# Hxyz-123/GoMatching

Measured on AMD Instinct MI355X. Metric: frames/sec (whole node), 1280x720 clip, 100 queries/frame, higher is better.
Workload: dtype f32 (f16x3 split MFMA: 22-bit significand products, fp32 accumulate; parity tests at fp32 tolerances)

## Files before the change

gomatching_amd/csrc/msda.hip:

```cpp
#include <mutex>
#include <type_traits>
#include <vector>

#include "common.h"

namespace {

constexpr int HEADS = 8, CH = 32, LEVELS = 4;

__device__ __forceinline__ long xcd_contiguous_block(unsigned bid, unsigned nwg) {
    const unsigned q = nwg >> 3, r = nwg & 7, xcd = bid & 7;
    return (long)(xcd < r ? xcd * (q + 1) : r * (q + 1) + (xcd - r) * q) + (bid >> 3);
}

template <int POINTS>
__global__ __launch_bounds__(256) void msda_fwd_kernel(const float* __restrict__ value,
                                                       const int64_t* __restrict__ shapes,
                                                       const int64_t* __restrict__ lsi,
                                                       const float* __restrict__ loc,
                                                       const float* __restrict__ attw, float* __restrict__ out,
                                                       int B, int Lq, long v_bs, int v_rs) {
    const long q_global = xcd_contiguous_block(blockIdx.x, gridDim.x) * 4 + (threadIdx.x >> 6);
    if (q_global >= (long)B * Lq) return;
    const int lane = threadIdx.x & 63;
// ... 247 lines not shown

    const __amdgpu_buffer_rsrc_t rs = gom_buffer_rsrc(value + (size_t)b * v_bs, 0x7FFFFFFF);
    const unsigned mine = (unsigned)k * 16u;
    f32x4 acc = {0.f, 0.f, 0.f, 0.f};
#pragma unroll
    for (int i = 0; i < LP; ++i) {
        const int o = i >> 1, t = i & 1;
        const unsigned a1 = __builtin_bit_cast(unsigned, group8_read(__builtin_bit_cast(float, so1[t]), o)) + mine;
        const unsigned a2 = __builtin_bit_cast(unsigned, group8_read(__builtin_bit_cast(float, so2[t]), o)) + mine;
        const unsigned a3 = __builtin_bit_cast(unsigned, group8_read(__builtin_bit_cast(float, so3[t]), o)) + mine;
        const unsigned a4 = __builtin_bit_cast(unsigned, group8_read(__builtin_bit_cast(float, so4[t]), o)) + mine;
        const f32x4 v1 = __builtin_bit_cast(f32x4, __builtin_amdgcn_raw_buffer_load_b128(rs, (int)a1, 0, 0));
        const f32x4 v2 = __builtin_bit_cast(f32x4, __builtin_amdgcn_raw_buffer_load_b128(rs, (int)a2, 0, 0));
        const f32x4 v3 = __builtin_bit_cast(f32x4, __builtin_amdgcn_raw_buffer_load_b128(rs, (int)a3, 0, 0));
        const f32x4 v4 = __builtin_bit_cast(f32x4, __builtin_amdgcn_raw_buffer_load_b128(rs, (int)a4, 0, 0));
        const float w1 = group8_read(sw1[t], o), w2 = group8_read(sw2[t], o), w3 = group8_read(sw3[t], o), w4 = group8_read(sw4[t], o);
        msda_fma4(acc, w1, v1);
        msda_fma4(acc, w2, v2);
        msda_fma4(acc, w3, v3);
        msda_fma4(acc, w4, v4);
    }
    *reinterpret_cast<f32x4*>(out + (size_t)q_global * (HEADS * CH) + m * CH + k * 4) = acc;
}

template <int R, int CAP>
__host__ __device__ __forceinline__ void msda_window_plan(const int (&Hs)[LEVELS], const int (&Ws)[LEVELS], float rxa, float rya,
                                                          float rxz, float ryz, int glv, int schedule, int (&wx0)[LEVELS],
                                                          int (&wy0)[LEVELS], int (&wx1)[LEVELS], int (&wy1)[LEVELS],
                                                          int (&wwd)[LEVELS], int (&wst)[LEVELS]) {
    static_assert(CAP % 8 == 0 && CAP >= 16, "regions are whole groups of 8 lines");
    const int first = glv == 0 ? 1 : 2;
    int split = 0;
#pragma unroll
    for (int i = 0; i < LEVELS; ++i) {
        int ax = (int)floorf(fminf(rxa, rxz) * Ws[i] - 0.5f) - R, zx = (int)floorf(fmaxf(rxa, rxz) * Ws[i] - 0.5f) + R + 1;
        int ay = (int)floorf(fminf(rya, ryz) * Hs[i] - 0.5f) - R, zy = (int)floorf(fmaxf(rya, ryz) * Hs[i] - 0.5f) + R + 1;
        ax = ax > 0 ? ax : 0; ay = ay > 0 ? ay : 0; zx = zx < Ws[i] - 1 ? zx : Ws[i] - 1; zy = zy < Hs[i] - 1 ? zy : Hs[i] - 1;
        if (zx < ax) zx = ax;
        if (zy < ay) zy = ay;
        int start = 0, cap = CAP;
        if (schedule == 1) {
            if (i == first) cap = CAP - 8;
            if (i == first + 1) { start = split; cap = CAP - split; }
            if (glv == 0 && i == 3) cap = split;
        }
        int w_ = zx - ax + 1, h_ = zy - ay + 1;
        if (w_ > cap) { w_ = cap; zx = ax + w_ - 1; }
        if (w_ * h_ > cap) { h_ = cap / w_; zy = ay + h_ - 1; }
        if (i == first) split = (w_ * h_ + 7) & ~7;
        wx0[i] = ax; wy0[i] = ay; wx1[i] = zx; wy1[i] = zy; wwd[i] = w_; wst[i] = start;
    }
}

template <int TY, int TX, int R, int CAP, int NB, int GLV = 0, int OVL = 0>
__global__ __launch_bounds__(256, 2) void msda_window_kernel(const float* __restrict__ value,
                                                             const int64_t* __restrict__ shapes,
                                                             const int64_t* __restrict__ lsi,
                                                             const float* __restrict__ raw, int ld_raw,
                                                             const float* __restrict__ ref, float* __restrict__ out,
                                                             int Lq, long v_bs, int v_rs, int tiles_y, int tiles_x, int ql,
                                                             unsigned* __restrict__ slow_groups) {
    constexpr int POINTS = 4, LP = LEVELS * POINTS, ITERS = (TY * TX) / 32;
    extern __shared__ __attribute__((aligned(16))) unsigned char win[];
    const int tid = threadIdx.x, lane = tid & 63;
    const int wave = __builtin_amdgcn_readfirstlane(tid >> 6);
    const int g = lane >> 3, k = lane & 7;
    const int m = (int)(blockIdx.x & 7u);
    unsigned tile = blockIdx.x >> 3;
    const int tx = (int)(tile % (unsigned)tiles_x);
    tile /= (unsigned)tiles_x;
    const int ty = (int)(tile % (unsigned)tiles_y);
    const int b = (int)(tile / (unsigned)tiles_y);
    const int l = k >> 1;

    int Hs[LEVELS], Ws[LEVELS];
    unsigned lv[LEVELS];
#pragma unroll
    for (int i = 0; i < LEVELS; ++i) {
        Hs[i] = (int)shapes[2 * i];
        Ws[i] = (int)shapes[2 * i + 1];
        lv[i] = (unsigned)lsi[i];
    }
    const int Hq = ql == 0 ? Hs[0] : ql == 1 ? Hs[1] : ql == 2 ? Hs[2] : Hs[3];
    const int Wq = ql == 0 ? Ws[0] : ql == 1 ? Ws[1] : ql == 2 ? Ws[2] : Ws[3];
    const long q0 = (long)b * Lq + (long)(ql == 0 ? lv[0] : ql == 1 ? lv[1] : ql == 2 ? lv[2] : lv[3]);
    const int y0t = ty * TY, x0t = tx * TX;
    const int y1t = min(y0t + TY, Hq) - 1, x1t = min(x0t + TX, Wq) - 1;
    const long qa = q0 + (long)y0t * Wq + x0t, qz = q0 + (long)y1t * Wq + x1t;
    const float rxa = ref[qa * 2], rya = ref[qa * 2 + 1], rxz = ref[qz * 2], ryz = ref[qz * 2 + 1];
    int wx0[LEVELS], wy0[LEVELS], wx1[LEVELS], wy1[LEVELS], wwd[LEVELS], wst[LEVELS];
    msda_window_plan<R, CAP>(Hs, Ws, rxa, rya, rxz, ryz, GLV, OVL, wx0, wy0, wx1, wy1, wwd, wst);
    const int H = l == 0 ? Hs[0] : l == 1 ? Hs[1] : l == 2 ? Hs[2] : Hs[3];
    const int W = l == 0 ? Ws[0] : l == 1 ? Ws[1] : l == 2 ? Ws[2] : Ws[3];
    const int mx0 = l == 0 ? wx0[0] : l == 1 ? wx0[1] : l == 2 ? wx0[2] : wx0[3];
    const int my0 = l == 0 ? wy0[0] : l == 1 ? wy0[1] : l == 2 ? wy0[2] : wy0[3];
    const int mx1 = l == 0 ? wx1[0] : l == 1 ? wx1[1] : l == 2 ? wx1[2] : wx1[3];
    const int my1 = l == 0 ? wy1[0] : l == 1 ? wy1[1] : l == 2 ? wy1[2] : wy1[3];
    const int mww = l == 0 ? wwd[0] : l == 1 ? wwd[1] : l == 2 ? wwd[2] : wwd[3];
    const int mst = l == 0 ? wst[0] : l == 1 ? wst[1] : l == 2 ? wst[2] : wst[3];
    const unsigned lvl = l == 0 ? lv[0] : l == 1 ? lv[1] : l == 2 ? lv[2] : lv[3];
    const float Hf = (float)H, Wf = (float)W;
    const float rW = 1.f / Wf, rH = 1.f / Hf;

    const __amdgpu_buffer_rsrc_t rs = gom_buffer_rsrc(value + (size_t)b * v_bs, 0x7FFFFFFF);
    const unsigned mine = (unsigned)k * 16u;
    const unsigned head = (unsigned)(m * CH) * 4u;

    float sw1[ITERS][2], sw2[ITERS][2], sw3[ITERS][2], sw4[ITERS][2];
    unsigned pk[ITERS][2];
    unsigned go1[GLV ? ITERS : 1][2], go2[GLV ? ITERS : 1][2], go3[GLV ? ITERS : 1][2], go4[GLV ? ITERS : 1][2];
    f32x4 acc[ITERS];
    long qrow[ITERS];
    bool fast[ITERS], live[ITERS];
    f32x4 offs[ITERS];
// ... 274 lines not shown
        }
#pragma unroll
        for (int it = 0; it < ITERS; ++it) {
            if (fast[it]) continue;
            const long q_global = qrow[it];
            const f32x4 off4 = *reinterpret_cast<const f32x4*>(raw + (size_t)q_global * ld_raw + m * (LP * 2) + 4 * k);
            const float* lp = raw + (size_t)q_global * ld_raw + HEADS * LP * 2 + m * LP + 2 * k;
            const float lg0 = lp[0], lg1 = lp[1];
            float mx = fmaxf(lg0, lg1);
            mx = fmaxf(mx, __builtin_bit_cast(float, __builtin_amdgcn_ds_swizzle(__builtin_bit_cast(int, mx), 0x1F | (1 << 10))));
            mx = fmaxf(mx, __builtin_bit_cast(float, __builtin_amdgcn_ds_swizzle(__builtin_bit_cast(int, mx), 0x1F | (2 << 10))));
            mx = fmaxf(mx, __builtin_bit_cast(float, __builtin_amdgcn_ds_swizzle(__builtin_bit_cast(int, mx), 0x1F | (4 << 10))));
            const float e0 = expf(lg0 - mx), e1 = expf(lg1 - mx);
            float sum = 0.f;
#pragma unroll
            for (int o = 0; o < 8; ++o) {
                sum += group8_read(e0, o);
                sum += group8_read(e1, o);
            }
            const float inv_sum = 1.f / sum;
            bool ok_;
            unsigned sa1, sa2, sa3, sa4, sb1, sb2, sb3, sb4;
            const float rx_ = ref[q_global * 2], ry_ = ref[q_global * 2 + 1];
            MSDA_GEOMETRY(it, 0, off4, rx_, ry_, e0, inv_sum, ok_, sa)
            MSDA_GEOMETRY(it, 1, off4, rx_, ry_, e1, inv_sum, ok_, sb)
            (void)ok_;
            f32x4 r = {0.f, 0.f, 0.f, 0.f};
#pragma unroll
            for (int i = 0; i < LP; ++i) {
                const int o = i >> 1, t = i & 1;
                const unsigned a1 = __builtin_bit_cast(unsigned, group8_read(__builtin_bit_cast(float, t ? sb1 : sa1), o)) + mine;
                const unsigned a2 = __builtin_bit_cast(unsigned, group8_read(__builtin_bit_cast(float, t ? sb2 : sa2), o)) + mine;
                const unsigned a3 = __builtin_bit_cast(unsigned, group8_read(__builtin_bit_cast(float, t ? sb3 : sa3), o)) + mine;
                const unsigned a4 = __builtin_bit_cast(unsigned, group8_read(__builtin_bit_cast(float, t ? sb4 : sa4), o)) + mine;
                const f32x4 v1 = __builtin_bit_cast(f32x4, __builtin_amdgcn_raw_buffer_load_b128(rs, (int)a1, 0, 0));
                const f32x4 v2 = __builtin_bit_cast(f32x4, __builtin_amdgcn_raw_buffer_load_b128(rs, (int)a2, 0, 0));
                const f32x4 v3 = __builtin_bit_cast(f32x4, __builtin_amdgcn_raw_buffer_load_b128(rs, (int)a3, 0, 0));
                const f32x4 v4 = __builtin_bit_cast(f32x4, __builtin_amdgcn_raw_buffer_load_b128(rs, (int)a4, 0, 0));
                const float w1 = group8_read(sw1[it][t], o), w2 = group8_read(sw2[it][t], o), w3 = group8_read(sw3[it][t], o),
                            w4 = group8_read(sw4[it][t], o);
                msda_fma4(r, w1, v1);
                msda_fma4(r, w2, v2);
                msda_fma4(r, w3, v3);
                msda_fma4(r, w4, v4);
            }
            acc[it] = r;
        }
    }
#pragma unroll
    for (int it = 0; it < ITERS; ++it)
        if (live[it]) *reinterpret_cast<f32x4*>(out + (size_t)qrow[it] * (HEADS * CH) + m * CH + k * 4) = acc[it];
}

#undef MSDA_GEOMETRY

}

static int g_msda_lanes = 1;
extern "C" int gom_msda_set_lane_distributed(int on) {
    g_msda_lanes = on ? 1 : 0;
    return GOM_OK;
}

extern "C" int gom_msda_fused_forward(const float* raw, int ld_raw, const float* ref, const float* value,
                                      long value_batch_stride, int value_row_stride, const int64_t* spatial_shapes,
                                      const int64_t* level_start_index, float* output, int batch, int num_query,
                                      void* stream) {
    GOM_CHECK_ARG(raw && ref && value && spatial_shapes && level_start_index && output);
    GOM_CHECK_ARG(batch > 0 && num_query > 0 && ld_raw >= HEADS * LEVELS * 4 * 3 && (ld_raw % 4) == 0);
    GOM_CHECK_ARG(value_row_stride >= HEADS * CH && (value_row_stride % 4) == 0 && (value_batch_stride % 4) == 0);
    GOM_CHECK_ARG(((uintptr_t)raw % 16) == 0 && ((uintptr_t)value % 16) == 0);
    const long nq = (long)batch * num_query;
    if (g_msda_lanes && value_batch_stride > 0 && value_batch_stride < (1L << 29))
        hipLaunchKernelGGL((msda_fused_lanes_kernel<0>), dim3((unsigned)cdiv(nq, 4)), dim3(256), 0, (hipStream_t)stream,
                           value, spatial_shapes, level_start_index, raw, ld_raw, ref, output, batch, num_query,
                           value_batch_stride, value_row_stride, (const float*)nullptr, 0, num_query);
    else
        hipLaunchKernelGGL((msda_fused_kernel<4, 0>), dim3((unsigned)cdiv(nq, 4)), dim3(256), 0, (hipStream_t)stream, value,
                           spatial_shapes, level_start_index, raw, ld_raw, ref, output, batch, num_query,
                           value_batch_stride, value_row_stride, (const float*)nullptr);
    return gom_launch_status();
}

static int g_msda_window = 7;
static unsigned* g_msda_slow = nullptr;
extern "C" int gom_msda_set_window(int mask) {
    g_msda_window = mask < 0 ? 0 : (mask & 7);
    return GOM_OK;
}
extern "C" int gom_msda_window_count_fallbacks(unsigned int* device_counter) {
    g_msda_slow = device_counter;
    return GOM_OK;
}

extern "C" int gom_msda_fused_forward_encoder(const float* raw, int ld_raw, const float* ref, const float* value,
                                              long value_batch_stride, int value_row_stride, const int64_t* spatial_shapes,
                                              const int64_t* level_start_index, float* output, int batch, int num_query,
                                              int h0, int w0, int h1, int w1, void* stream) {
    GOM_CHECK_ARG(raw && ref && value && spatial_shapes && level_start_index && output);
    GOM_CHECK_ARG(batch > 0 && num_query > 0 && ld_raw >= HEADS * LEVELS * 4 * 3 && (ld_raw % 4) == 0);
    GOM_CHECK_ARG(value_row_stride >= HEADS * CH && (value_row_stride % 4) == 0 && (value_batch_stride % 4) == 0);
    GOM_CHECK_ARG(((uintptr_t)raw % 16) == 0 && ((uintptr_t)value % 16) == 0);
    GOM_CHECK_ARG(h0 > 0 && w0 > 0 && h1 >= 0 && w1 >= 0 && (long)h0 * w0 + (long)h1 * w1 <= num_query);
    constexpr int R = 5, CAP = 576;
    constexpr int TY0 = 8, TX0 = 16, TY1 = 8, TX1 = 16;
    const long n0 = (long)h0 * w0, n1 = (long)h1 * w1;
    const long wgs0 = (long)batch * cdiv(h0, TY0) * cdiv(w0, TX0) * 8;
    const long wgs1 = (long)batch * cdiv(h1, TY1) * cdiv(w1, TX1) * 8;
    if (!((g_msda_window & 1) && g_msda_lanes && value_batch_stride > 0 && value_batch_stride < (1L << 29) && wgs0 < (1L << 31) &&
          wgs1 < (1L << 31)))
        return gom_msda_fused_forward(raw, ld_raw, ref, value, value_batch_stride, value_row_stride, spatial_shapes,
                                      level_start_index, output, batch, num_query, stream);
    hipStream_t s = (hipStream_t)stream;
    const bool ovl = (g_msda_window & 4) != 0;
    {
        auto kern = ovl ? msda_window_kernel<TY0, TX0, R, CAP, 4, 0, 1> : msda_window_kernel<TY0, TX0, R, CAP, 4, 0, 0>;
        hipError_t e = hipFuncSetAttribute((const void*)kern, hipFuncAttributeMaxDynamicSharedMemorySize, CAP * 128);
        if (e != hipSuccess) return GOM_ERR_HIP_BASE + (int)e;
        hipLaunchKernelGGL(kern, dim3((unsigned)wgs0), dim3(256), CAP * 128, s, value, spatial_shapes, level_start_index, raw, ld_raw,
                           ref, output, num_query, value_batch_stride, value_row_stride, cdiv(h0, TY0), cdiv(w0, TX0), 0, g_msda_slow);
    }
    long done = n0;
    if ((g_msda_window & 2) && n1 > 0) {
        auto kern = ovl ? msda_window_kernel<TY1, TX1, R, CAP, 4, 1, 1> : msda_window_kernel<TY1, TX1, R, CAP, 4, 1, 0>;
        hipError_t e = hipFuncSetAttribute((const void*)kern, hipFuncAttributeMaxDynamicSharedMemorySize, CAP * 128);
        if (e != hipSuccess) return GOM_ERR_HIP_BASE + (int)e;
        hipLaunchKernelGGL(kern, dim3((unsigned)wgs1), dim3(256), CAP * 128, s, value, spatial_shapes, level_start_index, raw, ld_raw,
                           ref, output, num_query, value_batch_stride, value_row_stride, cdiv(h1, TY1), cdiv(w1, TX1), 1, g_msda_slow);
        done += n1;
    }
    const long rest = num_query - done;
    if (rest > 0)
        hipLaunchKernelGGL((msda_fused_lanes_kernel<0>), dim3((unsigned)cdiv((long)batch * rest, 4)), dim3(256), 0, s, value,
                           spatial_shapes, level_start_index, raw, ld_raw, ref, output, batch, num_query, value_batch_stride,
                           value_row_stride, (const float*)nullptr, (int)done, (int)rest);
    return gom_launch_status();
}

extern "C" int gom_msda_window_plan(const int64_t* spatial_shapes, int tile_level, const float* ref_first, const float* ref_last,
                                    int schedule, int* plan, int* cap_lines) {
    GOM_CHECK_ARG(spatial_shapes && ref_first && ref_last && plan && cap_lines);
    GOM_CHECK_ARG((tile_level == 0 || tile_level == 1) && (schedule == 0 || schedule == 1));
    constexpr int R = 5, CAP = 576;
    int Hs[LEVELS], Ws[LEVELS], wx0[LEVELS], wy0[LEVELS], wx1[LEVELS], wy1[LEVELS], wwd[LEVELS], wst[LEVELS];
    for (int i = 0; i < LEVELS; ++i) {
        GOM_CHECK_ARG(spatial_shapes[2 * i] > 0 && spatial_shapes[2 * i + 1] > 0);
        Hs[i] = (int)spatial_shapes[2 * i];
        Ws[i] = (int)spatial_shapes[2 * i + 1];
    }
    msda_window_plan<R, CAP>(Hs, Ws, ref_first[0], ref_first[1], ref_last[0], ref_last[1], tile_level, schedule, wx0, wy0, wx1, wy1,
                             wwd, wst);
    for (int i = 0; i < LEVELS; ++i) {
        const bool gathered = i < tile_level;
        plan[3 * i] = gathered ? 0 : wst[i];
        plan[3 * i + 1] = gathered ? 0 : wwd[i];
        plan[3 * i + 2] = gathered ? 0 : wy1[i] - wy0[i] + 1;
    }
    *cap_lines = CAP;
    return GOM_OK;
}

extern "C" int gom_msda_fused_forward_vr(const float* raw, int ld_raw, const float* ref, const float* value,
                                         long value_batch_stride, int value_row_stride, const int64_t* spatial_shapes,
                                         const int64_t* level_start_index, const float* valid_ratios, float* output,
                                         int batch, int num_query, void* stream) {
    GOM_CHECK_ARG(raw && ref && value && spatial_shapes && level_start_index && valid_ratios && output);
    GOM_CHECK_ARG(batch > 0 && num_query > 0 && ld_raw >= HEADS * LEVELS * 4 * 3 && (ld_raw % 4) == 0);
    GOM_CHECK_ARG(value_row_stride >= HEADS * CH && (value_row_stride % 4) == 0 && (value_batch_stride % 4) == 0);
    GOM_CHECK_ARG(((uintptr_t)raw % 16) == 0 && ((uintptr_t)value % 16) == 0);
    const long nq = (long)batch * num_query;
    if (g_msda_lanes && value_batch_stride > 0 && value_batch_stride < (1L << 29))
        hipLaunchKernelGGL((msda_fused_lanes_kernel<1>), dim3((unsigned)cdiv(nq, 4)), dim3(256), 0, (hipStream_t)stream,
                           value, spatial_shapes, level_start_index, raw, ld_raw, ref, output, batch, num_query,
                           value_batch_stride, value_row_stride, valid_ratios, 0, num_query);
    else
        hipLaunchKernelGGL((msda_fused_kernel<4, 1>), dim3((unsigned)cdiv(nq, 4)), dim3(256), 0, (hipStream_t)stream, value,
                           spatial_shapes, level_start_index, raw, ld_raw, ref, output, batch, num_query,
// ... 68 lines not shown
```

gomatching_amd/ops.py:

```python
import collections
import contextlib
import ctypes
import math

import numpy as np
import torch

from . import lib as _lib_mod
from .lib import check

_f32 = torch.float32


def _L():
    return _lib_mod.load()


_gemm_profile = None


_profile_scope = ""


@contextlib.contextmanager
# ... 960 lines not shown
    code, dims = _msda_args(value, spatial_shapes, level_start_index, sampling_loc, attn_weight)
    B, S, M, D, Lv, Lq, Pn = dims
    out = torch.empty((B, Lq, M * D), dtype=value.dtype, device=value.device)
    if code == 0:
        check(_L().gom_ms_deform_attn_forward(_p(value), _p(spatial_shapes), _p(level_start_index), _p(sampling_loc),
                                              _p(attn_weight), _p(out), B, S, M, D, Lv, Lq, Pn, _stream()),
              "gom_ms_deform_attn_forward")
    else:
        check(_L().gom_ms_deform_attn_forward_any(code, _p(value), _p(spatial_shapes), _p(level_start_index), _p(sampling_loc),
                                                  _p(attn_weight), _p(out), B, S, M, D, Lv, Lq, Pn, _stream()),
              "gom_ms_deform_attn_forward_any")
    return out


def ms_deform_attn_forward_any(value, spatial_shapes, level_start_index, sampling_loc, attn_weight):
    code, dims = _msda_args(value, spatial_shapes, level_start_index, sampling_loc, attn_weight)
    B, S, M, D, Lv, Lq, Pn = dims
    out = torch.empty((B, Lq, M * D), dtype=value.dtype, device=value.device)
    check(_L().gom_ms_deform_attn_forward_any(code, _p(value), _p(spatial_shapes), _p(level_start_index), _p(sampling_loc),
                                              _p(attn_weight), _p(out), B, S, M, D, Lv, Lq, Pn, _stream()),
          "gom_ms_deform_attn_forward_any")
    return out


def ms_deform_attn_backward(value, spatial_shapes, level_start_index, sampling_loc, attn_weight, grad_output, im2col_step=64):
    code, dims = _msda_args(value, spatial_shapes, level_start_index, sampling_loc, attn_weight, grad_output)
    B, S, M, D, Lv, Lq, Pn = dims
    if grad_output.numel() != B * Lq * M * D:
        raise _lib_mod.GomError("ms_deform_attn_backward: grad_output must hold [B, Lq, M*D] elements")
    gv, gl, gw = torch.empty_like(value), torch.empty_like(sampling_loc), torch.empty_like(attn_weight)
    check(_L().gom_ms_deform_attn_backward(code, _p(value), _p(spatial_shapes), _p(level_start_index), _p(sampling_loc),
                                           _p(attn_weight), _p(grad_output), _p(gv), _p(gl), _p(gw), B, S, M, D, Lv, Lq, Pn,
                                           _stream()),
          "gom_ms_deform_attn_backward")
    return gv, gl, gw


def ms_deform_attn_forward_strided(value2d, batch_stride, shapes, lsi, loc, w, B, Lq):
    assert value2d.stride(1) == 1
    out = torch.empty((B * Lq, 256), dtype=_f32, device=value2d.device)
    check(_L().gom_ms_deform_attn_forward_strided(_p(value2d), batch_stride, value2d.stride(0), _p(shapes), _p(lsi),
                                                  _p(loc), _p(w), _p(out), B, Lq, _stream()),
          "gom_ms_deform_attn_forward_strided")
    return out


MSDA_LANES = _switch("MSDA_LANES")
_msda_lanes_set = [None]


MSDA_WINDOW = _switch("MSDA_WINDOW")
MSDA_WINDOW_L1 = _switch("MSDA_WINDOW_L1")
MSDA_WINDOW_OVERLAP = _switch("MSDA_WINDOW_OVERLAP")
_msda_window_set = [None]


MSDA_WINDOW_POLICY = _switch("MSDA_WINDOW_POLICY")
MSDA_WINDOW_MAX_FALLBACK = 0.30


def msda_window_groups(encoder_hw0, B):
    h0, w0 = int(encoder_hw0[0]), int(encoder_hw0[1])
    n = -(-h0 // 8) * -(-w0 // 16) * 16
    if MSDA_WINDOW_L1 and len(encoder_hw0) >= 4:
        n += -(-int(encoder_hw0[2]) // 8) * -(-int(encoder_hw0[3]) // 16) * 16
    return B * 8 * n


def msda_fused(raw, ref, value2d, batch_stride, shapes, lsi, B, Lq, valid_ratios=None, encoder_hw0=None, fallback_counter=None,
               frame_valid_ratios=None):
    assert raw.stride(1) == 1 and value2d.stride(1) == 1
    _chk_f32(ref, valid_ratios)
    if frame_valid_ratios is not None:
        assert valid_ratios is None, "valid_ratios and frame_valid_ratios are exclusive"
        _chk_frame_desc(frame_valid_ratios, B, (shapes.shape[0], 2), _f32, "frame_valid_ratios")
    if _msda_lanes_set[0] != MSDA_LANES:
        _L().gom_msda_set_lane_distributed(1 if MSDA_LANES else 0)
        _msda_lanes_set[0] = MSDA_LANES
    out = torch.empty((B * Lq, 256), dtype=_f32, device=raw.device)
    S_rows = value2d.shape[0]
    with _timed(True, lambda: (2.0 * B * Lq * 8 * 16 * 4 * 32, 4.0 * (S_rows * 256 + B * Lq * (384 + 256)), "msda:%dx%d" % (B, Lq))):
        if frame_valid_ratios is not None:
            check(_L().gom_msda_fused_forward_vr_frames(_p(raw), raw.stride(0), _p(ref), _p(value2d), batch_stride,
                                                        value2d.stride(0), _p(shapes), _p(lsi), _p(frame_valid_ratios), _p(out),
                                                        B, Lq, _stream()), "gom_msda_fused_forward_vr_frames")
        elif valid_ratios is not None:
            check(_L().gom_msda_fused_forward_vr(_p(raw), raw.stride(0), _p(ref), _p(value2d), batch_stride,
                                                 value2d.stride(0), _p(shapes), _p(lsi), _p(valid_ratios), _p(out), B, Lq,
                                                 _stream()), "gom_msda_fused_forward_vr")
        elif encoder_hw0 is not None and MSDA_WINDOW and MSDA_LANES:
            mask = (3 if MSDA_WINDOW_L1 else 1) | (4 if MSDA_WINDOW_OVERLAP else 0)
            if _msda_window_set[0] != mask:
                _L().gom_msda_set_window(mask)
                _msda_window_set[0] = mask
            h1, w1 = (int(encoder_hw0[2]), int(encoder_hw0[3])) if len(encoder_hw0) >= 4 else (0, 0)
            if fallback_counter is not None:
                fallback_counter.zero_()
                _L().gom_msda_window_count_fallbacks(_p(fallback_counter))
            try:
                check(_L().gom_msda_fused_forward_encoder(_p(raw), raw.stride(0), _p(ref), _p(value2d), batch_stride, value2d.stride(0),
                                                          _p(shapes), _p(lsi), _p(out), B, Lq, int(encoder_hw0[0]), int(encoder_hw0[1]),
                                                          h1, w1, _stream()), "gom_msda_fused_forward_encoder")
            finally:
                if fallback_counter is not None:
                    _L().gom_msda_window_count_fallbacks(None)
        else:
            check(_L().gom_msda_fused_forward(_p(raw), raw.stride(0), _p(ref), _p(value2d), batch_stride, value2d.stride(0),
                                              _p(shapes), _p(lsi), _p(out), B, Lq, _stream()), "gom_msda_fused_forward")
    return out


def msda_prepare(raw, ref, spatial_shapes, ref_levels=1):
    _chk_f32(ref)
    Q = raw.shape[0]
    loc = torch.empty((Q, 8, 4, 4, 2), dtype=_f32, device=raw.device)
    w = torch.empty((Q, 8, 4, 4), dtype=_f32, device=raw.device)
    check(_L().gom_msda_prepare(_p(raw), raw.stride(0), _p(ref), ref_levels, _p(spatial_shapes), _p(loc), _p(w), Q,
                                _stream()), "gom_msda_prepare")
    return loc, w


def mha_core(q, k, v, out, outer, inner, heads, head_dim, Lq, Lk, strides):
    arr = (ctypes.c_long * 12)(*[int(s) for s in strides])
    check(_L().gom_mha_core_f32(_p(q), _p(k), _p(v), _p(out), outer, inner, heads, head_dim, Lq, Lk, arr, _stream()),
          "gom_mha_core_f32")
    return out


def mha_core_segments(q, k, v, out, segments, num_segments, heads, head_dim, ld_q, ld_k, ld_v, ld_o, max_Lq, max_Lk):
    check(_L().gom_mha_core_segments_f32(_p(q), _p(k), _p(v), _p(out), _p(segments), num_segments, heads, head_dim,
                                         ld_q, ld_k, ld_v, ld_o, max_Lq, max_Lk, _stream()), "gom_mha_core_segments_f32")
    return out


def preprocess(images, mean, std):
    _chk_f32(images)
    B, C, H, W = images.shape
    assert C == 3
    out = torch.empty((B, H, W, 4), dtype=_f32, device=images.device)
    m = (ctypes.c_float * 3)(*[float(v) for v in mean])
    s = (ctypes.c_float * 3)(*[float(v) for v in std])
    check(_L().gom_preprocess_nchw_to_nhwc4(_p(images), m, s, _p(out), B, H, W, _stream()), "gom_preprocess")
    return out

# ... 1059 lines not shown
```

Baseline: 313.6.

## Add four-lanes-per-query layout for windowed MSDA encoder kernel

Adds a variant of the windowed deformable-attention kernel in which each query-head uses four lanes (one per level), each covering eight channels, instead of eight lanes of four channels. Weights and packed LDS offsets are shared across the quad with DPP reads, and each lane issues two 128-bit LDS reads per corner. The variant has selectable channel-assignment schemes meant to avoid bank conflicts. The aim is to halve the per-lane softmax and geometry work and process more queries per wave, at the cost of more registers and DPP shuffles. It is enabled for the level-0 kernel through a new mask bit and a Python switch.

```diff
diff --git a/gomatching_amd/csrc/msda.hip b/gomatching_amd/csrc/msda.hip
--- a/gomatching_amd/csrc/msda.hip
+++ b/gomatching_amd/csrc/msda.hip
@@ -323,7 +323,13 @@
     }
 }
 
-template <int TY, int TX, int R, int CAP, int NB, int GLV = 0, int OVL = 0>
+template <int TY, int TX, int R, int CAP, int NB, int GLV, int OVL, int CHA>
+__device__ __forceinline__ void msda_window_lanes4(const float* __restrict__ value, const int64_t* __restrict__ shapes,
+                                                   const int64_t* __restrict__ lsi, const float* __restrict__ raw, int ld_raw,
+                                                   const float* __restrict__ ref, float* __restrict__ out, int Lq, long v_bs, int v_rs,
+                                                   int tiles_y, int tiles_x, int ql, unsigned* __restrict__ slow_groups);
+
+template <int TY, int TX, int R, int CAP, int NB, int GLV = 0, int OVL = 0, int LPQ = 8, int CHA = 0>
 __global__ __launch_bounds__(256, 2) void msda_window_kernel(const float* __restrict__ value,
                                                              const int64_t* __restrict__ shapes,
                                                              const int64_t* __restrict__ lsi,
@@ -331,6 +337,12 @@
                                                              const float* __restrict__ ref, float* __restrict__ out,
                                                              int Lq, long v_bs, int v_rs, int tiles_y, int tiles_x, int ql,
                                                              unsigned* __restrict__ slow_groups) {
+    static_assert(LPQ == 8 || LPQ == 4, "two lane layouts");
+    if constexpr (LPQ == 4) {
+        msda_window_lanes4<TY, TX, R, CAP, NB, GLV, OVL, CHA>(value, shapes, lsi, raw, ld_raw, ref, out, Lq, v_bs, v_rs, tiles_y, tiles_x,
+                                                              ql, slow_groups);
+        return;
+    }
     constexpr int POINTS = 4, LP = LEVELS * POINTS, ITERS = (TY * TX) / 32;
     extern __shared__ __attribute__((aligned(16))) unsigned char win[];
     const int tid = threadIdx.x, lane = tid & 63;
@@ -711,6 +723,390 @@
         if (live[it]) *reinterpret_cast<f32x4*>(out + (size_t)qrow[it] * (HEADS * CH) + m * CH + k * 4) = acc[it];
 }
 
+__device__ __forceinline__ float quad_read(float v, int owner) {
+    const int x = __builtin_bit_cast(int, v);
+    switch (owner) {
+        case 0: return __builtin_bit_cast(float, __builtin_amdgcn_mov_dpp(x, 0x00, 0xF, 0xF, true));
+        case 1: return __builtin_bit_cast(float, __builtin_amdgcn_mov_dpp(x, 0x55, 0xF, 0xF, true));
+        case 2: return __builtin_bit_cast(float, __builtin_amdgcn_mov_dpp(x, 0xAA, 0xF, 0xF, true));
+        default: return __builtin_bit_cast(float, __builtin_amdgcn_mov_dpp(x, 0xFF, 0xF, 0xF, true));
+    }
+}
+__device__ __forceinline__ unsigned quad_read(unsigned v, int owner) {
+    return __builtin_bit_cast(unsigned, quad_read(__builtin_bit_cast(float, v), owner));
+}
+
+template <int TY, int TX, int R, int CAP, int NB, int GLV, int OVL, int CHA>
+__device__ __forceinline__ void msda_window_lanes4(const float* __restrict__ value, const int64_t* __restrict__ shapes,
+                                                   const int64_t* __restrict__ lsi, const float* __restrict__ raw, int ld_raw,
+                                                   const float* __restrict__ ref, float* __restrict__ out, int Lq, long v_bs, int v_rs,
+                                                   int tiles_y, int tiles_x, int ql, unsigned* __restrict__ slow_groups) {
+    constexpr int POINTS = 4, LP = LEVELS * POINTS, ITERS = (TY * TX) / 64;
+    static_assert((TY * TX) % 64 == 0 && ITERS % NB == 0, "whole iterations of 16 queries per wave, whole batches");
+    static_assert(8 * NB <= 16, "lgkmcnt counts to 15");
+    static_assert(CHA >= 0 && CHA <= 2, "three channel assignments");
+    static_assert(GLV == 0 || GLV == 1, "only the finest level is ever gathered");
+    static_assert(OVL == 0 || OVL == 1, "two fill schedules");
+    extern __shared__ __attribute__((aligned(16))) unsigned char win[];
+    const int tid = threadIdx.x, lane = tid & 63;
+    const int wave = __builtin_amdgcn_readfirstlane(tid >> 6);
+    const int g = lane >> 3, k = lane & 7;
+    const int p16 = lane >> 2, l = lane & 3;
+    const int m = (int)(blockIdx.x & 7u);
+    unsigned tile = blockIdx.x >> 3;
+    const int tx = (int)(tile % (unsigned)tiles_x);
+    tile /= (unsigned)tiles_x;
+    const int ty = (int)(tile % (unsigned)tiles_y);
+    const int b = (int)(tile / (unsigned)tiles_y);
+
+    int Hs[LEVELS], Ws[LEVELS];
+    unsigned lv[LEVELS];
+#pragma unroll
+    for (int i = 0; i < LEVELS; ++i) {
+        Hs[i] = (int)shapes[2 * i];
+        Ws[i] = (int)shapes[2 * i + 1];
+        lv[i] = (unsigned)lsi[i];
+    }
+    const int Hq = ql == 0 ? Hs[0] : ql == 1 ? Hs[1] : ql == 2 ? Hs[2] : Hs[3];
+    const int Wq = ql == 0 ? Ws[0] : ql == 1 ? Ws[1] : ql == 2 ? Ws[2] : Ws[3];
+    const long q0 = (long)b * Lq + (long)(ql == 0 ? lv[0] : ql == 1 ? lv[1] : ql == 2 ? lv[2] : lv[3]);
+    const int y0t = ty * TY, x0t = tx * TX;
+    const int y1t = min(y0t + TY, Hq) - 1, x1t = min(x0t + TX, Wq) - 1;
+    const long qa = q0 + (long)y0t * Wq + x0t, qz = q0 + (long)y1t * Wq + x1t;
+    const float rxa = ref[qa * 2], rya = ref[qa * 2 + 1], rxz = ref[qz * 2], ryz = ref[qz * 2 + 1];
+    int wx0[LEVELS], wy0[LEVELS], wx1[LEVELS], wy1[LEVELS], wwd[LEVELS], wst[LEVELS];
+    msda_window_plan<R, CAP>(Hs, Ws, rxa, rya, rxz, ryz, GLV, OVL, wx0, wy0, wx1, wy1, wwd, wst);
+    const int H = l == 0 ? Hs[0] : l == 1 ? Hs[1] : l == 2 ? Hs[2] : Hs[3];
+    const int W = l == 0 ? Ws[0] : l == 1 ? Ws[1] : l == 2 ? Ws[2] : Ws[3];
+    const int mx0 = l == 0 ? wx0[0] : l == 1 ? wx0[1] : l == 2 ? wx0[2] : wx0[3];
+    const int my0 = l == 0 ? wy0[0] : l == 1 ? wy0[1] : l == 2 ? wy0[2] : wy0[3];
+    const int mx1 = l == 0 ? wx1[0] : l == 1 ? wx1[1] : l == 2 ? wx1[2] : wx1[3];
+    const int my1 = l == 0 ? wy1[0] : l == 1 ? wy1[1] : l == 2 ? wy1[2] : wy1[3];
+    const int mww = l == 0 ? wwd[0] : l == 1 ? wwd[1] : l == 2 ? wwd[2] : wwd[3];
+    const int mst = l == 0 ? wst[0] : l == 1 ? wst[1] : l == 2 ? wst[2] : wst[3];
+    const unsigned lvl = l == 0 ? lv[0] : l == 1 ? lv[1] : l == 2 ? lv[2] : lv[3];
+    const float Hf = (float)H, Wf = (float)W;
+    const float rW = 1.f / Wf, rH = 1.f / Hf;
+
+    const __amdgpu_buffer_rsrc_t rs = gom_buffer_rsrc(value + (size_t)b * v_bs, 0x7FFFFFFF);
+    const unsigned head = (unsigned)(m * CH) * 4u;
+    constexpr unsigned SECOND = CHA == 0 ? 16u : 64u;
+    const unsigned flip = CHA == 2 ? (unsigned)((lane >> 3) & 1) : 0u;
+    const unsigned mine = CHA == 0 ? (unsigned)l * 32u : (unsigned)l * 16u + flip * 64u;
+    const unsigned mine2 = CHA == 2 ? (unsigned)l * 16u + (1u - flip) * 64u : mine + SECOND;
+
+    float sw1[ITERS][4], sw2[ITERS][4], sw3[ITERS][4], sw4[ITERS][4];
+    unsigned pk[ITERS][4];
+    unsigned go1[GLV ? ITERS : 1][4], go2[GLV ? ITERS : 1][4], go3[GLV ? ITERS : 1][4], go4[GLV ? ITERS : 1][4];
+    f32x4 acc[ITERS][2];
+    long qrow[ITERS];
+    bool fast[ITERS][2], live[ITERS];
+    f32x4 offa[ITERS], offb[ITERS], lgs[ITERS];
+    float rxs[ITERS], rys[ITERS];
+#pragma unroll
+    for (int it = 0; it < ITERS; ++it) {
+        const int j = (wave * ITERS + it) * 16 + p16;
+        const int jy = j / TX, jx = j - jy * TX;
+        const int qy = y0t + jy, qx = x0t + jx;
+        live[it] = qy <= y1t && qx <= x1t;
+        const long q_global = q0 + (long)(live[it] ? qy : y0t) * Wq + (live[it] ? qx : x0t);
+        qrow[it] = q_global;
+        const float* op = raw + (size_t)q_global * ld_raw + m * (LP * 2) + 8 * l;
+        const float* lp = raw + (size_t)q_global * ld_raw + HEADS * LP * 2 + m * LP + 4 * l;
+        offa[it] = *reinterpret_cast<const f32x4*>(op);
+        offb[it] = *reinterpret_cast<const f32x4*>(op + 4);
+        lgs[it] = *reinterpret_cast<const f32x4*>(lp);
+        rxs[it] = ref[q_global * 2];
+        rys[it] = ref[q_global * 2 + 1];
+    }
+    auto fill = [&](auto LEVC) {
+        constexpr int lev = decltype(LEVC)::value;
+        unsigned char* buf = win + (size_t)wst[lev] * 128;
+        const int ww_ = wwd[lev], n_lines = ww_ * (wy1[lev] - wy0[lev] + 1);
+        const float inv_w = 1.f / (float)ww_;
+        for (int base = wave * 8; base < n_lines; base += 32) {
+            int line = base + g;
+            if (line > n_lines - 1) line = n_lines - 1;
+            int yy = (int)(((float)line + 0.5f) * inv_w);
+            int xx = line - yy * ww_;
+            if (xx < 0) { --yy; xx += ww_; }
+            if (xx >= ww_) { ++yy; xx -= ww_; }
+            const unsigned src = (lv[lev] + (unsigned)((wy0[lev] + yy) * Ws[lev] + wx0[lev] + xx)) * (unsigned)v_rs * 4u + head + (unsigned)k * 16u;
+            __builtin_amdgcn_raw_ptr_buffer_load_lds(rs, (__attribute__((address_space(3))) void*)(buf + (size_t)base * 128), 16,
+                                                     (int)src, 0, 0, 0);
+        }
+    };
+    if constexpr (OVL != 0) {
+#pragma unroll
+        for (int it = 0; it < ITERS; ++it) asm volatile("" : "+v"(offa[it]), "+v"(offb[it]), "+v"(lgs[it]), "+v"(rxs[it]), "+v"(rys[it]));
+        fill(std::integral_constant<int, GLV>{});
+    }
+    unsigned any_slow = 0;
+#pragma unroll
+    for (int it = 0; it < ITERS; ++it) {
+        const f32x4 lg = lgs[it];
+        float mx = fmaxf(fmaxf(lg[0], lg[1]), fmaxf(lg[2], lg[3]));
+        mx = fmaxf(mx, __builtin_bit_cast(float, __builtin_amdgcn_mov_dpp(__builtin_bit_cast(int, mx), 0xB1, 0xF, 0xF, true)));
+        mx = fmaxf(mx, __builtin_bit_cast(float, __builtin_amdgcn_mov_dpp(__builtin_bit_cast(int, mx), 0x4E, 0xF, 0xF, true)));
+        float e[POINTS];
+#pragma unroll
+        for (int t = 0; t < POINTS; ++t) e[t] = expf(lg[t] - mx);
+        float sum = 0.f;
+#pragma unroll
+        for (int o = 0; o < LEVELS; ++o)
+#pragma unroll
+            for (int t = 0; t < POINTS; ++t) sum += quad_read(e[t], o);
+        const float inv_sum = 1.f / sum;
+        const float off8[8] = {offa[it][0], offa[it][1], offa[it][2], offa[it][3], offb[it][0], offb[it][1], offb[it][2], offb[it][3]};
+        bool ok0, ok1, ok2, ok3;
+        unsigned sa1, sa2, sa3, sa4, sb1, sb2, sb3, sb4, sc1, sc2, sc3, sc4, sd1, sd2, sd3, sd4;
+        MSDA_GEOMETRY(it, 0, off8, rxs[it], rys[it], e[0], inv_sum, ok0, sa)
+        MSDA_GEOMETRY(it, 1, off8, rxs[it], rys[it], e[1], inv_sum, ok1, sb)
+        MSDA_GEOMETRY(it, 2, off8, rxs[it], rys[it], e[2], inv_sum, ok2, sc)
+        MSDA_GEOMETRY(it, 3, off8, rxs[it], rys[it], e[3], inv_sum, ok3, sd)
+        if constexpr (GLV > 0) {
+            go1[it][0] = sa1; go2[it][0] = sa2; go3[it][0] = sa3; go4[it][0] = sa4;
+            go1[it][1] = sb1; go2[it][1] = sb2; go3[it][1] = sb3; go4[it][1] = sb4;
+            go1[it][2] = sc1; go2[it][2] = sc2; go3[it][2] = sc3; go4[it][2] = sc4;
+            go1[it][3] = sd1; go2[it][3] = sd2; go3[it][3] = sd3; go4[it][3] = sd4;
+        }
+        (void)sa1; (void)sa2; (void)sa3; (void)sa4; (void)sb1; (void)sb2; (void)sb3; (void)sb4;
+        (void)sc1; (void)sc2; (void)sc3; (void)sc4; (void)sd1; (void)sd2; (void)sd3; (void)sd4;
+        const unsigned long long bad = __builtin_amdgcn_ballot_w64(!(ok0 && ok1 && ok2 && ok3));
+        fast[it][0] = (unsigned)bad == 0u;
+        fast[it][1] = (unsigned)(bad >> 32) == 0u;
+        any_slow |= (fast[it][0] && fast[it][1]) ? 0u : 1u;
+        acc[it][0] = f32x4{0.f, 0.f, 0.f, 0.f};
+        acc[it][1] = f32x4{0.f, 0.f, 0.f, 0.f};
+    }
+
+    auto level_samples = [&](auto LEVC) {
+        constexpr int lev = decltype(LEVC)::value;
+        const unsigned mine_lds = mine + (unsigned)(size_t)win;
+        const unsigned row_bytes = (unsigned)wwd[lev] * 128u;
+#pragma unroll
+        for (int t = 0; t < POINTS; ++t) {
+#pragma unroll
+            for (int half = 0; half < ITERS; half += NB) {
+                bool any_fast = false;
+#pragma unroll
+                for (int u = 0; u < NB; ++u) any_fast = any_fast || fast[half + u][0] || fast[half + u][1];
+                if (!any_fast) continue;
+                unsigned word[NB];
+                float w1[NB], w2[NB], w3[NB], w4[NB];
+#pragma unroll
+                for (int u = 0; u < NB; ++u) {
+                    const int it = half + u;
+                    asm volatile("" : "+v"(pk[it][t]), "+v"(sw1[it][t]), "+v"(sw2[it][t]), "+v"(sw3[it][t]), "+v"(sw4[it][t]));
+                    word[u] = quad_read(pk[it][t], lev);
+                    w1[u] = quad_read(sw1[it][t], lev);
+                    w2[u] = quad_read(sw2[it][t], lev);
+                    w3[u] = quad_read(sw3[it][t], lev);
+                    w4[u] = quad_read(sw4[it][t], lev);
+                }
+                f32x4 va[NB][4], vb[NB][4];
+#pragma unroll
+                for (int u = 0; u < NB; ++u) {
+                    const unsigned a1 = (word[u] & 0xFFFFFu) + mine_lds;
+                    const unsigned dx = (word[u] >> 20) & 1u, dy = (word[u] >> 21) & 1u;
+                    unsigned a[4] = {a1, a1 + dx * 128u, a1 + dy * row_bytes, 0u};
+                    a[3] = a[2] + dx * 128u;
+                    asm volatile("" : "+v"(a[1]), "+v"(a[2]), "+v"(a[3]));
+#pragma unroll
+                    for (int c = 0; c < 4; ++c) {
+                        asm volatile("ds_read_b128 %0, %1" : "=&v"(va[u][c]) : "v"(a[c]));
+                        if constexpr (CHA == 2) {
+                            const unsigned a_ = a[c] + (mine2 - mine);
+                            asm volatile("ds_read_b128 %0, %1" : "=&v"(vb[u][c]) : "v"(a_));
+                        } else {
+                            asm volatile("ds_read_b128 %0, %1 offset:%2" : "=&v"(vb[u][c]) : "v"(a[c]), "n"(SECOND));
+                        }
+                    }
+                }
+#pragma unroll
+                for (int u = 0; u < NB; ++u) {
+                    const float w[4] = {w1[u], w2[u], w3[u], w4[u]};
+#pragma unroll
+                    for (int c = 0; c < 4; ++c) {
+                        asm volatile("s_waitcnt lgkmcnt(%2)" : "+v"(va[u][c]), "+v"(vb[u][c]) : "n"(8 * NB - 2 - (8 * u + 2 * c)));
+                        msda_fma4(acc[half + u][0], w[c], va[u][c]);
+                        msda_fma4(acc[half + u][1], w[c], vb[u][c]);
+                    }
+                }
+                __builtin_amdgcn_sched_barrier(0);
+            }
+        }
+    };
+    auto level_gather = [&](auto LEVC) {
+        constexpr int lev = decltype(LEVC)::value;
+#pragma unroll
+        for (int t = 0; t < POINTS; ++t) {
+#pragma unroll
+            for (int half = 0; half < ITERS; half += NB) {
+                bool any_fast = false;
+#pragma unroll
+                for (int u = 0; u < NB; ++u) any_fast = any_fast || fast[half + u][0] || fast[half + u][1];
+                if (!any_fast) continue;
+                unsigned a[NB][4];
+                float w[NB][4];
+#pragma unroll
+                for (int u = 0; u < NB; ++u) {
+                    const int it = half + u;
+                    asm volatile("" : "+v"(go1[it][t]), "+v"(go2[it][t]), "+v"(go3[it][t]), "+v"(go4[it][t]));
+                    asm volatile("" : "+v"(sw1[it][t]), "+v"(sw2[it][t]), "+v"(sw3[it][t]), "+v"(sw4[it][t]));
+                    a[u][0] = quad_read(go1[it][t], lev);
+                    a[u][1] = quad_read(go2[it][t], lev);
+                    a[u][2] = quad_read(go3[it][t], lev);
+                    a[u][3] = quad_read(go4[it][t], lev);
+                    w[u][0] = quad_read(sw1[it][t], lev);
+                    w[u][1] = quad_read(sw2[it][t], lev);
+                    w[u][2] = quad_read(sw3[it][t], lev);
+                    w[u][3] = quad_read(sw4[it][t], lev);
+                }
+                f32x4 va[NB][4], vb[NB][4];
+#pragma unroll
+                for (int u = 0; u < NB; ++u)
+#pragma unroll
+                    for (int c = 0; c < 4; ++c) {
+                        va[u][c] = __builtin_bit_cast(f32x4, __builtin_amdgcn_raw_buffer_load_b128(rs, (int)(a[u][c] + mine), 0, 0));
+                        vb[u][c] = __builtin_bit_cast(f32x4, __builtin_amdgcn_raw_buffer_load_b128(rs, (int)(a[u][c] + mine2), 0, 0));
+                    }
+#pragma unroll
+                for (int u = 0; u < NB; ++u)
+#pragma unroll
+                    for (int c = 0; c < 4; ++c) {
+                        msda_fma4(acc[half + u][0], w[u][c], va[u][c]);
+                        msda_fma4(acc[half + u][1], w[u][c], vb[u][c]);
+                    }
+                __builtin_amdgcn_sched_barrier(0);
+            }
+        }
+    };
+    auto landed = [] {
+        asm volatile("s_waitcnt vmcnt(0)" ::: "memory");
+        __syncthreads();
+    };
+    auto level_single = [&](auto LEVC) {
+        __syncthreads();
+        fill(LEVC);
+        landed();
+        level_samples(LEVC);
+    };
+    typedef std::integral_constant<int, 0> L0;
+    typedef std::integral_constant<int, 1> L1;
+    typedef std::integral_constant<int, 2> L2;
+    typedef std::integral_constant<int, 3> L3;
+    if constexpr (OVL == 0 && GLV == 0) {
+        level_single(L0{});
+        level_single(L1{});
+        level_single(L2{});
+        level_single(L3{});
+    } else if constexpr (OVL == 0) {
+        fill(L1{});
+        level_gather(L0{});
+        landed();
+        level_samples(L1{});
+        level_single(L2{});
+        level_single(L3{});
+    } else if constexpr (GLV == 0) {
+#pragma unroll
+        for (int it = 0; it < ITERS; ++it)
+#pragma unroll
+            for (int t = 0; t < POINTS; ++t)
+                asm volatile("" ::"v"(pk[it][t]), "v"(sw1[it][t]), "v"(sw2[it][t]), "v"(sw3[it][t]), "v"(sw4[it][t]));
+        __builtin_amdgcn_sched_barrier(0);
+        landed();
+        level_samples(L0{});
+        __syncthreads();
+        fill(L1{});
+        fill(L2{});
+        landed();
+        level_samples(L1{});
+        __syncthreads();
+        fill(L3{});
+        level_samples(L2{});
+        landed();
+        level_samples(L3{});
+    } else {
+        level_gather(L0{});
+        landed();
+        level_samples(L1{});
+        __syncthreads();
+        fill(L2{});
+        fill(L3{});
+        landed();
+        level_samples(L2{});
+        level_samples(L3{});
+    }
+    if (any_slow) {
+        if (slow_groups && lane == 0) {
+            unsigned n_slow = 0;
+#pragma unroll
+            for (int it = 0; it < ITERS; ++it) n_slow += (fast[it][0] ? 0u : 1u) + (fast[it][1] ? 0u : 1u);
+            atomicAdd(slow_groups, n_slow);
+        }
+#pragma unroll
+        for (int it = 0; it < ITERS; ++it) {
+            const bool slow_here = lane < 32 ? !fast[it][0] : !fast[it][1];
+            if (!slow_here) continue;
+            const long q_global = qrow[it];
+            const float* op = raw + (size_t)q_global * ld_raw + m * (LP * 2) + 8 * l;
+            const f32x4 oa = *reinterpret_cast<const f32x4*>(op), ob = *reinterpret_cast<const f32x4*>(op + 4);
+            const f32x4 lg = *reinterpret_cast<const f32x4*>(raw + (size_t)q_global * ld_raw + HEADS * LP * 2 + m * LP + 4 * l);
+            float mx = fmaxf(fmaxf(lg[0], lg[1]), fmaxf(lg[2], lg[3]));
+            mx = fmaxf(mx, __builtin_bit_cast(float, __builtin_amdgcn_mov_dpp(__builtin_bit_cast(int, mx), 0xB1, 0xF, 0xF, true)));
+            mx = fmaxf(mx, __builtin_bit_cast(float, __builtin_amdgcn_mov_dpp(__builtin_bit_cast(int, mx), 0x4E, 0xF, 0xF, true)));
+            float e[POINTS];
+#pragma unroll
+            for (int t = 0; t < POINTS; ++t) e[t] = expf(lg[t] - mx);
+            float sum = 0.f;
+#pragma unroll
+            for (int o = 0; o < LEVELS; ++o)
+#pragma unroll
+                for (int t = 0; t < POINTS; ++t) sum += quad_read(e[t], o);
+            const float inv_sum = 1.f / sum;
+            const float off8[8] = {oa[0], oa[1], oa[2], oa[3], ob[0], ob[1], ob[2], ob[3]};
+            bool ok_;
+            unsigned sa1, sa2, sa3, sa4, sb1, sb2, sb3, sb4, sc1, sc2, sc3, sc4, sd1, sd2, sd3, sd4;
+            const float rx_ = ref[q_global * 2], ry_ = ref[q_global * 2 + 1];
+            MSDA_GEOMETRY(it, 0, off8, rx_, ry_, e[0], inv_sum, ok_, sa)
+            MSDA_GEOMETRY(it, 1, off8, rx_, ry_, e[1], inv_sum, ok_, sb)
+            MSDA_GEOMETRY(it, 2, off8, rx_, ry_, e[2], inv_sum, ok_, sc)
+            MSDA_GEOMETRY(it, 3, off8, rx_, ry_, e[3], inv_sum, ok_, sd)
+            (void)ok_;
+            const unsigned s1[4] = {sa1, sb1, sc1, sd1}, s2[4] = {sa2, sb2, sc2, sd2}, s3[4] = {sa3, sb3, sc3, sd3},
+                           s4[4] = {sa4, sb4, sc4, sd4};
+            f32x4 ra = {0.f, 0.f, 0.f, 0.f}, rb = {0.f, 0.f, 0.f, 0.f};
+#pragma unroll
+            for (int i = 0; i < LP; ++i) {
+                const int o = i >> 2, t = i & 3;
+                const unsigned a[4] = {quad_read(s1[t], o), quad_read(s2[t], o), quad_read(s3[t], o), quad_read(s4[t], o)};
+                const float w[4] = {quad_read(sw1[it][t], o), quad_read(sw2[it][t], o), quad_read(sw3[it][t], o), quad_read(sw4[it][t], o)};
+                f32x4 va[4], vb[4];
+#pragma unroll
+                for (int c = 0; c < 4; ++c) {
+                    va[c] = __builtin_bit_cast(f32x4, __builtin_amdgcn_raw_buffer_load_b128(rs, (int)(a[c] + mine), 0, 0));
+                    vb[c] = __builtin_bit_cast(f32x4, __builtin_amdgcn_raw_buffer_load_b128(rs, (int)(a[c] + mine2), 0, 0));
+                }
+#pragma unroll
+                for (int c = 0; c < 4; ++c) {
+                    msda_fma4(ra, w[c], va[c]);
+                    msda_fma4(rb, w[c], vb[c]);
+                }
+            }
+            acc[it][0] = ra;
+            acc[it][1] = rb;
+        }
+    }
+#pragma unroll
+    for (int it = 0; it < ITERS; ++it)
+        if (live[it]) {
+            float* o_ = out + (size_t)qrow[it] * (HEADS * CH) + m * CH;
+            *reinterpret_cast<f32x4*>(o_ + (mine >> 2)) = acc[it][0];
+            *reinterpret_cast<f32x4*>(o_ + (mine2 >> 2)) = acc[it][1];
+        }
+}
+
 #undef MSDA_GEOMETRY
 
 }
@@ -741,10 +1137,31 @@
     return gom_launch_status();
 }
 
-static int g_msda_window = 7;
+#ifndef MSDA_LANES4_L0
+#define MSDA_LANES4_L0 1
+#endif
+#ifndef MSDA_LANES4_L1
+#define MSDA_LANES4_L1 0
+#endif
+#ifndef MSDA_LANES4_CHA
+#define MSDA_LANES4_CHA 2
+#endif
+typedef void (*msda_window_fn)(const float*, const int64_t*, const int64_t*, const float*, int, const float*, float*, int, long, int, int,
+                               int, int, unsigned*);
+template <int TY, int TX, int R, int CAP, int GLV, int KEPT4>
+static msda_window_fn msda_window_pick(bool ovl, bool lanes4) {
+    if constexpr (KEPT4 != 0) {
+        if (lanes4)
+            return ovl ? msda_window_kernel<TY, TX, R, CAP, 2, GLV, 1, 4, MSDA_LANES4_CHA>
+                       : msda_window_kernel<TY, TX, R, CAP, 2, GLV, 0, 4, MSDA_LANES4_CHA>;
+    }
+    return ovl ? msda_window_kernel<TY, TX, R, CAP, 4, GLV, 1> : msda_window_kernel<TY, TX, R, CAP, 4, GLV, 0>;
+}
+
+static int g_msda_window = 15;
 static unsigned* g_msda_slow = nullptr;
 extern "C" int gom_msda_set_window(int mask) {
-    g_msda_window = mask < 0 ? 0 : (mask & 7);
+    g_msda_window = mask < 0 ? 0 : (mask & 15);
     return GOM_OK;
 }
 extern "C" int gom_msda_window_count_fallbacks(unsigned int* device_counter) {
@@ -771,9 +1188,9 @@
         return gom_msda_fused_forward(raw, ld_raw, ref, value, value_batch_stride, value_row_stride, spatial_shapes,
                                       level_start_index, output, batch, num_query, stream);
     hipStream_t s = (hipStream_t)stream;
-    const bool ovl = (g_msda_window & 4) != 0;
+    const bool ovl = (g_msda_window & 4) != 0, l4 = (g_msda_window & 8) != 0;
     {
-        auto kern = ovl ? msda_window_kernel<TY0, TX0, R, CAP, 4, 0, 1> : msda_window_kernel<TY0, TX0, R, CAP, 4, 0, 0>;
+        auto kern = msda_window_pick<TY0, TX0, R, CAP, 0, MSDA_LANES4_L0>(ovl, l4);
         hipError_t e = hipFuncSetAttribute((const void*)kern, hipFuncAttributeMaxDynamicSharedMemorySize, CAP * 128);
         if (e != hipSuccess) return GOM_ERR_HIP_BASE + (int)e;
         hipLaunchKernelGGL(kern, dim3((unsigned)wgs0), dim3(256), CAP * 128, s, value, spatial_shapes, level_start_index, raw, ld_raw,
@@ -781,7 +1198,7 @@
     }
     long done = n0;
     if ((g_msda_window & 2) && n1 > 0) {
-        auto kern = ovl ? msda_window_kernel<TY1, TX1, R, CAP, 4, 1, 1> : msda_window_kernel<TY1, TX1, R, CAP, 4, 1, 0>;
+        auto kern = msda_window_pick<TY1, TX1, R, CAP, 1, MSDA_LANES4_L1>(ovl, l4);
         hipError_t e = hipFuncSetAttribute((const void*)kern, hipFuncAttributeMaxDynamicSharedMemorySize, CAP * 128);
         if (e != hipSuccess) return GOM_ERR_HIP_BASE + (int)e;
         hipLaunchKernelGGL(kern, dim3((unsigned)wgs1), dim3(256), CAP * 128, s, value, spatial_shapes, level_start_index, raw, ld_raw,
diff --git a/gomatching_amd/ops.py b/gomatching_amd/ops.py
--- a/gomatching_amd/ops.py
+++ b/gomatching_amd/ops.py
@@ -1036,6 +1036,7 @@
 MSDA_WINDOW = _switch("MSDA_WINDOW")
 MSDA_WINDOW_L1 = _switch("MSDA_WINDOW_L1")
 MSDA_WINDOW_OVERLAP = _switch("MSDA_WINDOW_OVERLAP")
+MSDA_WINDOW_LANES4 = _switch("MSDA_WINDOW_LANES4")
 _msda_window_set = [None]
 
 
@@ -1073,7 +1074,7 @@
                                                  value2d.stride(0), _p(shapes), _p(lsi), _p(valid_ratios), _p(out), B, Lq,
                                                  _stream()), "gom_msda_fused_forward_vr")
         elif encoder_hw0 is not None and MSDA_WINDOW and MSDA_LANES:
-            mask = (3 if MSDA_WINDOW_L1 else 1) | (4 if MSDA_WINDOW_OVERLAP else 0)
+            mask = (3 if MSDA_WINDOW_L1 else 1) | (4 if MSDA_WINDOW_OVERLAP else 0) | (8 if MSDA_WINDOW_LANES4 else 0)
             if _msda_window_set[0] != mask:
                 _L().gom_msda_set_window(mask)
                 _msda_window_set[0] = mask
```

Result: faster. 318.0 (median of 6 runs) (+1.4%).
